# vmskisme/f_renderer

Measured on AMD Instinct MI355X. Metric: Mtri/s (and Mfrag/s), 1M-triangle frame @1920x1080, higher is better.
Workload: dtype f32; 1 GPU; random_1M_tris_1920x1080_depth; scene=1M random clip-space triangles, 1920x1080, depth-only, width=1920, height=1080, triangles=1000000, setup_triangles=1000052, covered_fragments=60715175, varyings=0, tile=32x32, frames_in_flight=2, partition=tile rows in 1 contiguous block(s)

## Files before the change

f_renderer_amd/_native.py:

```python
import ctypes as C
import os
import shutil
import subprocess

_HERE = os.path.dirname(os.path.abspath(__file__))
_ROOT = os.path.dirname(_HERE)
LIB_PATH = os.environ.get("FRR_LIB") or os.path.join(_HERE, "libfrr_hip.so")
_SRC = [os.path.join(_HERE, "csrc", f) for f in ("frr_api.hip", "frr_kernels.h", "frr_raster.h", "frr_device.h", "frr_exact.h", "frr_tile_order.h", "frr_rules.h", "frr_proof.h", "frr_lines.h", "frr_varyings.h", "frr_shade.h", "frr_visible.h", "frr_query.h", "frr_boxes.h", "frr_own.h")]
_HDR = os.path.join(_ROOT, "include", "frr.h")

HIPCC_FLAGS = [
    "--offload-arch=gfx950", "-O3", "-std=c++17", "-fPIC", "-shared",
    "-ffp-contract=off", "-fno-fast-math", "-Wall", "-Wno-unused-function",
    "-fno-slp-vectorize",
    "-DFRR_CSRC_DIR=\"%s\"" % os.path.join(_HERE, "csrc"), "-L/opt/rocm/lib", "-lhiprtc", "-Wl,-rpath,/opt/rocm/lib",
]

FRR_OK, FRR_ERR_INVALID, FRR_ERR_HIP, FRR_ERR_NOMEM, FRR_ERR_UNSUPPORTED, FRR_ERR_CAPACITY = 0, -1, -2, -3, -4, -5
VS_CLIP, VS_CLIP_COLOR, VS_PHONG, VS_GOURAUD = 0, 1, 2, 3
PS_DEPTH, PS_FLAT, PS_COLOR, PS_PHONG, PS_BLINN = 0, 1, 2, 3, 4
CULL_NONE, CULL_NEG, CULL_POS = 0, 1, 2
PER_ITEM, PER_TRIANGLE = 0, 1
VISIBLE_LDS_BINS = 4096
MAX_VARYINGS = 16
# ... 190 lines not shown
```

f_renderer_amd/csrc/frr_api.hip:

```cpp
#include "frr_kernels.h"
#include "frr_tile_order.h"
#include "frr_rules.h"
#include "frr_proof.h"
#include "frr_lines.h"
#include "frr_varyings.h"
#include "frr_shade.h"
#include "frr_visible.h"
#include "frr_query.h"
#include "frr_boxes.h"
#include "frr_own.h"

#include <math.h>
#include <stdio.h>
#include <string.h>
#include <stdlib.h>

#include <hip/hiprtc.h>

#include <map>
#include <mutex>
#include <string>
#include <type_traits>
#include <vector>

// ... 6 lines not shown
FRR_EMBED(frr_src_exact_h, "frr_exact.h");
FRR_EMBED(frr_src_kernels_h, "frr_kernels.h");
FRR_EMBED(frr_src_raster_h, "frr_raster.h");
FRR_EMBED(frr_src_shade_h, "frr_shade.h");
FRR_EMBED(frr_src_visible_h, "frr_visible.h");
FRR_EMBED(frr_src_frr_h, "../../include/frr.h");
#endif
extern "C" const char frr_src_device_h[], frr_src_exact_h[], frr_src_kernels_h[], frr_src_raster_h[], frr_src_shade_h[], frr_src_visible_h[], frr_src_frr_h[];

using namespace frr;
static_assert(PASS_FAN_BITS == FAN_BITS && MAX_PASS_INPUTS << FAN_BITS == 1ull << PASS_ORDER_KEY_BITS, "frr_rules.h: an input's order keys are 32 * input + (0 .. 31), in 32 bits (frr_device.h)");

namespace {

enum KernelId { KID_CLEAR, KID_GEOM, KID_GEOM_SCAN, KID_BIN_COUNT,
                KID_TILE_SCAN, KID_BIN_FILL, KID_RASTER, KID_BIN_SEG, KID_LINES_MARK, KID_LINES_PAINT, KID_VISIBLE, KID_BOXES, KID_COUNT };
const char *const kKernelNames[KID_COUNT] = {"k_clear", "k_geom", "k_geom_scan",
                                             "k_bin_count", "k_tile_scan", "k_bin_fill",
                                             "k_raster", "k_bin_seg", "k_lines_mark", "k_lines_paint", "k_visible", "k_boxes"};

struct Mesh {
    DevBuf<float> own_dev; DevBuf<uint32_t> own_idx;
    const float *dev = nullptr;
    const uint32_t *idx = nullptr;
    uint64_t nverts = 0, ntris = 0;
    bool used = false;
    int vs = 0;
    uint64_t gen = 0;
};
struct Texture {
    DevBuf<uint8_t> dev;
    uint32_t w = 0, h = 0;
};
struct Lines {
// ... 106 lines not shown
    DevBuf<uint4> pbox;
    DevBuf<uint32_t> bcount;
    DevBuf<uint2> clipq;
    DevBuf<float> inst_tab;
    DevBuf<uint32_t> keep_tab;
    DevBuf<uint32_t> vslot[2]; hipStream_t vslot_stream[2] = {nullptr, nullptr};
    uint32_t vslot_seq[2] = {0, 0}, vslot_epoch[2] = {0, 0};
    ReaderFence reader;
};
struct BinSet {
    DevBuf<uint4> bins;
    DevBuf<uint4> bins2;
    DevBuf<uint32_t> bin_matrix;
    DevBuf<uint32_t> tile_cost;
    DevBuf<uint32_t> tile_perm;
    bool cost_known = false; TileOrderKey cost_key = {};
    ReaderFence reader;
};


struct Bound {
    uint8_t *color = nullptr; float *depth = nullptr; uint32_t *tri_id = nullptr;
    int tset = 0;
    int rank = 0, world = 1; bool part_blocked = false;
};
struct Clear {
    bool pending = false;
    bool unowned_debt = false;
    int debt_tiles_y = 0;
    uint32_t rgba = 0; float depth = 0.0f;
// ... 135 lines not shown
    uint32_t lines_chunk = 0;
    DevBuf<uint32_t> vis_bounds[3];
    uint32_t visible_lds_bins = 0;
    DevBuf<uint32_t> box_pyr[3];
    uint32_t box_bounds_chunks = 0;
    ReaderFence wire_reader[2];
    std::map<int, UserModule> user_modules;
    Texture tex[FRR_MAX_TEXTURES];
    frr_uniforms uni;
    DevUniforms duni;
    bool count_frags = true;
    int raster_nw = 0;
    int raster_occ = 0;
    bool raster_sweep = false;
    int tile_order = TILE_ORDER_FIXED;
    uint64_t ordered_passes = 0;
#ifdef FRR_DEBUG_COUNTERS
    DevBuf<unsigned long long> dbg_tiles;
#endif
    Event ev[16];
    bool ev_set[16] = {};
    uint32_t prof_mask = 0;
    std::vector<ProfRec> prof_pending;
    std::vector<Event> ev_pool;
    uint32_t prof_period = 1;
    uint32_t prof_seen[KID_COUNT] = {};
    double prof_ms[KID_COUNT] = {};
    uint32_t prof_n[KID_COUNT] = {};
    std::string err;
};
// ... 636 lines not shown
    a.tiles_x = (int)((ww + TILE - 1) / TILE); a.tiles_y = (int)((wh + TILE - 1) / TILE);
    a.tiles_x_magic = 0u;
    a.own = row_owner(f, a.tiles_y);
    a.recs = S.recs; a.vary = S.vary; a.pbox = S.pbox; a.bcount = S.bcount;
    a.tinfo = S.tinfo; a.fanbase = S.fanbase; a.fan_okey = S.fan_okey; a.block_prefix = S.block_prefix; a.ntris_draw = (uint32_t)f.geom.read.ntris;
    a.tile_counts = c->tile_counts; a.tile_offsets = c->tile_offsets; a.tile_cursor = c->tile_cursor;
    a.gpar = f.gpar(); a.lane = f.lane; a.bpar = 0; a.seq = cmd.seq; a.epoch = c->epoch; a.frame_no = f.frame_no; a.geom_seq = f.geom.seq;
    const uint32_t ntiles = (uint32_t)a.tiles_x * a.tiles_y;
    a.color = f.bound.color; a.depth = f.bound.depth; a.tri_id = f.bound.tri_id; a.cnt = c->cnt;
#ifdef FRR_DEBUG_COUNTERS
    if (!c->dbg_tiles && getenv("FRR_DEBUG_TILES")) (void)c->dbg_tiles.reset((size_t)c->max_tiles * 8);
    if (c->dbg_tiles) (void)hipMemsetAsync(c->dbg_tiles, 0, (size_t)c->max_tiles * 64, tstream_of(c));
    a.dbg_tiles = c->dbg_tiles;
#endif
    a.seg = nullptr; a.nseg = 0;
    a.tile_perm = nullptr; a.tile_cost = nullptr;
    const int owned_rows = a.own.blocked ? a.own.brow1 - a.own.brow0 : (a.tiles_y > f.bound.rank ? (a.tiles_y - f.bound.rank + f.bound.world - 1) / f.bound.world : 0);
    const uint32_t grid = (uint32_t)a.tiles_x * owned_rows;
    if (a.tiles_x >= 2 && a.tiles_x < 65536 && grid < 65536u) a.tiles_x_magic = (uint32_t)(0x100000000ull / (uint64_t)a.tiles_x + 1ull);
    const SpanShape sh = span_shape(c, grid, f.geom.read.ntris, ps_id);
    const bool segmented = grid <= BIN_LDS_MAX_TILES && !c->bin_atomics && !c->raster_sweep;
    const int q = segmented ? (f.bpar() ^ 1) : 0;
    const int bi = !segmented ? 0 : f.geom.on_g ? (f.bset ^ 1) : (frames_alternate(c) ? f.bound.tset : 0);
    BinSet &B = c->bset[bi];
    int rc;
    if (!B.bins) {
        size_t want = std::max<size_t>((size_t)f.geom.read.ntris * 8 + 4 * (size_t)c->max_tiles, (size_t)1 << 22);
        if (c->bin_cap_init) want = c->bin_cap_init;
        want = std::max(want, c->bset[bi ^ 1].bins.cap());
        if ((rc = ensure(c, B.bins, want)) != FRR_OK) return rc;
        if ((rc = ensure(c, B.bins2, want)) != FRR_OK) return rc;
    }
    a.bins2 = B.bins2;
    a.bins = B.bins; a.bin_cap = (uint32_t)std::min<size_t>(B.bins.cap(), 0xFFFFFFFFu);
    hipStream_t gs = gstream_of(c);
    if (segmented) {
        const uint32_t ltiles = std::max<uint32_t>(grid, 1u);
        uint32_t G = (uint32_t)std::min<uint64_t>(std::max<uint64_t>((f.geom.read.ntris + BIN_WG - 1) / BIN_WG, 1), BIN_MAX_G);
        if (c->bin_g > 0) G = (uint32_t)std::min(c->bin_g, BIN_MAX_G);
        G = std::min<uint32_t>(G, sh.nw == 3 ? 256u : (uint32_t)sh.nw * 64u);
        bool fresh_cost;
        if ((rc = ensure(c, B.tile_cost, ltiles, &fresh_cost)) != FRR_OK) return rc;
        if ((rc = ensure(c, B.tile_perm, ltiles)) != FRR_OK) return rc;
        if (fresh_cost) {
            B.cost_known = false;
            HIP_TRY(c, hipMemsetAsync(B.tile_cost, 0, (size_t)ltiles * sizeof(uint32_t), gs));
        }
        const TileOrderKey okey = {grid, a.tiles_x, x0, x1, y0, y1, f.bound.rank, f.bound.world, a.own.blocked, sh.nw};
        const bool ordered = tile_order_built(c->tile_order, c->in_replay, okey, B.cost_known, B.cost_key);
// ... 15 lines not shown
        }
        a.seg = B.bin_matrix; a.nseg = G; a.bpar = q;
        uint64_t SL = std::max<uint64_t>(256, (f.geom.read.ntris * 16 + ntiles - 1) / ntiles);
        SL = std::min<uint64_t>(SL, ((uint64_t)1 << 30) / ltiles);
        if (c->ent_slot_override) SL = c->ent_slot_override;
        a.ent_slot = (uint32_t)SL;
        a.bin_cap = (uint32_t)std::min<size_t>(B.bins.cap(), 0xBFFFFFFFu);
        if ((rc = ensure(c, B.bins2, (size_t)ltiles * SL + a.bin_cap)) != FRR_OK) return rc;
        a.bins2 = B.bins2;
        if ((rc = gstream_wait_readers(c, B.reader)) != FRR_OK) return rc;
        {
            ProfScope p(c, KID_BIN_SEG, gs);
            hipLaunchKernelGGL(k_bin_seg, dim3(G + extra), dim3(BIN_WG), lds, gs, a, ltiles, B.bin_matrix, stage_cap,
                               f.geom.fan_cap, S.block_sums, S.block_prefix, f.geom.nblocks, do_scan | (cmd.query ? 2 : 0), perm_seed);
        }
        if (!cmd.query) { B.cost_known = record; B.cost_key = okey; }
        if (ordered) ++c->ordered_passes;
        f.geom.scan_pending = false;
        f.bpars[f.lane] = q; f.bset = bi;
    } else {
        for (GeomSet &G2 : c->gset) if ((rc = gstream_wait_readers(c, G2.reader)) != FRR_OK) return rc;
        for (BinSet &B2 : c->bset) if ((rc = gstream_wait_readers(c, B2.reader)) != FRR_OK) return rc;
        if ((rc = scan_now(c)) != FRR_OK) return rc;
        const uint32_t bin_grid = (uint32_t)std::min<uint64_t>((f.geom.read.ntris + f.geom.fan_cap + 255) / 256, 2048);
        { ProfScope p(c, KID_BIN_COUNT, gs); hipLaunchKernelGGL(k_bin<false>, dim3(bin_grid), dim3(256), 0, gs, a, f.geom.fan_cap); }
        { ProfScope p(c, KID_TILE_SCAN, gs); if (cmd.query) hipLaunchKernelGGL(k_tile_scan_uncounted, dim3(1), dim3(1024), 0, gs, a, ntiles); else hipLaunchKernelGGL(k_tile_scan, dim3(1), dim3(1024), 0, gs, a, ntiles); }
        { ProfScope p(c, KID_BIN_FILL, gs); hipLaunchKernelGGL(k_bin<true>, dim3(bin_grid), dim3(256), 0, gs, a, f.geom.fan_cap); }
    }
    cmd.par = q; cmd.set = bi; cmd.lane = f.lane;
    HIP_TRY(c, hipGetLastError());
    if (!c->in_replay) {
        const DrawSig sig = draw_sig(f.geom.read, x0, x1, y0, y1, f.bound.rank, f.bound.world, f.bound.part_blocked, f.geom.set, bi, c->join_epoch);
        if (!c->proven.known(sig, f.geom.pred)) {
            HIP_TRY(c, hipEventRecord(c->ev_verify, gs));
            c->verify_pending = true;
            c->verify_pred = f.geom.pred;
            c->verify_sig = sig;
        }
    }
    if ((rc = tstream_wait_gstream(c)) != FRR_OK) return rc;
    if (cmd.query) return launch_query(c, cmd, a, grid, sh, S, B);
    hipStream_t ts;
    if ((rc = target_write(c, !c->in_replay, &ts)) != FRR_OK) return rc;
    const bool shared_entries = ww > (int64_t)x1 && f.bound.world <= 1;
    const int win_safe = a.x0 >= -SPAN_SAFE && a.y0 >= -SPAN_SAFE && a.x1 <= SPAN_SAFE && a.y1 <= SPAN_SAFE;
    if (grid && shared_entries) {
        ProfScope p(c, KID_RASTER, ts);
        const unsigned eg = (unsigned)((((wh - 1) * (int64_t)x1 + ww) + 255) / 256);
        if (um) {
            RasterArgs ra = a; DevUniforms d = cmd.duni;
            void *args[] = {&ra, &d};
            (void)hipModuleLaunchKernel(um->entries, eg, 1, 1, 256, 1, 1, 0, ts, args, nullptr);
        } else {
            switch (ps_id) {
            case FRR_PS_DEPTH: hipLaunchKernelGGL((k_raster_entries<0, FRR_PS_DEPTH>), dim3(eg), dim3(256), 0, ts, a, cmd.duni); break;
            case FRR_PS_FLAT: hipLaunchKernelGGL((k_raster_entries<0, FRR_PS_FLAT>), dim3(eg), dim3(256), 0, ts, a, cmd.duni); break;
            case FRR_PS_COLOR: hipLaunchKernelGGL((k_raster_entries<3, FRR_PS_COLOR>), dim3(eg), dim3(256), 0, ts, a, cmd.duni); break;
            case FRR_PS_PHONG: hipLaunchKernelGGL((k_raster_entries<8, FRR_PS_PHONG>), dim3(eg), dim3(256), 0, ts, a, cmd.duni); break;
            case FRR_PS_BLINN: hipLaunchKernelGGL((k_raster_entries<8, FRR_PS_BLINN>), dim3(eg), dim3(256), 0, ts, a, cmd.duni); break;
            }
// ... 571 lines not shown
    { int rc = finish(c); if (rc != FRR_OK) return rc; }
    c->proven.clear();
    const std::string n(name);
    if (n == "raster_sweep") c->raster_sweep = v != 0;
    else if (n == "raster_nw") { if (v != 0 && v != LIGHT_NW && v != 4 && v != 6 && v != 8 && v != 16) return fail(c, FRR_ERR_INVALID, "raster_nw: 0, 3, 4, 6, 8 or 16"); c->raster_nw = (int)v; }
    else if (n == "raster_occ") { if (v != 0 && v != 4 && v != 6 && v != 8) return fail(c, FRR_ERR_INVALID, "raster_occ: 0, 4, 6 or 8"); c->raster_occ = (int)v; }
    else if (n == "bin_chunks") { if (v < 0) return fail(c, FRR_ERR_INVALID, "bin_chunks >= 0"); c->bin_g = (int)std::min<int64_t>(v, BIN_MAX_G); }
    else if (n == "clear_eager") c->clear_eager = v != 0;
    else if (n == "clip_queue") { if (v < -1 || v > 1) return fail(c, FRR_ERR_INVALID, "clip_queue: -1, 0 or 1"); c->clip_queue = (int)v; }
    else if (n == "tile_slot_records") { if (v < 0 || v > 0x7FFFFFFF) return fail(c, FRR_ERR_INVALID, "tile_slot_records out of range"); c->ent_slot_override = (uint32_t)v; }
    else if (n == "bin_atomics") c->bin_atomics = v != 0;
    else if (n == "bin_capacity") { if (v < 0) return fail(c, FRR_ERR_INVALID, "bin_capacity >= 0"); c->bin_cap_init = (size_t)v; }
    else if (n == "fan_capacity") { if (v < 0) return fail(c, FRR_ERR_INVALID, "fan_capacity >= 0"); c->fan_cap_init = (size_t)v; }
    else if (n == "overlap") { if (v < 0 || v > 2) return fail(c, FRR_ERR_INVALID, "overlap: 0, 1 or 2"); c->overlap = (int)v; }
    else if (n == "bound_targets_in_flight") c->bound_in_flight = v != 0;
    else if (n == "tile_order") { if (v < 0 || v > 2) return fail(c, FRR_ERR_INVALID, "tile_order: 0, 1 or 2"); c->tile_order = (int)v; }
    else if (n == "box_bounds_chunks") { if (v < 0 || v > 1024) return fail(c, FRR_ERR_INVALID, "box_bounds_chunks: 0 .. 1024"); c->box_bounds_chunks = (uint32_t)v; }
    else if (n == "visible_lds_bins") { if (v < 0 || v > (int64_t)VIS_LDS_BINS) return fail(c, FRR_ERR_INVALID, "visible_lds_bins: 0 .. VIS_LDS_BINS"); c->visible_lds_bins = (uint32_t)v; }
    else if (n == "lines_chunk") { if (v < 0 || v > (int64_t)LINES_CHUNK) return fail(c, FRR_ERR_INVALID, "lines_chunk: 0 .. 2^24"); c->lines_chunk = (uint32_t)v; }
    else if (n == "frames_in_flight") { if (v != 1 && v != 2) return fail(c, FRR_ERR_INVALID, "frames_in_flight: 1 or 2"); c->frames_in_flight = (int)v; }
    else return fail(c, FRR_ERR_INVALID, "unknown option");
    return FRR_OK;
}

int frr_set_partition(frr_ctx *c, int rank, int world)
{
    if (!c || world < 1 || rank < 0 || rank >= world) return fail(c, FRR_ERR_INVALID, "bad partition");
    { int rc = settle(c); if (rc != FRR_OK) return rc; }
    c->fs.bound.rank = rank; c->fs.bound.world = world;
    return FRR_OK;
// ... 1363 lines not shown
```

f_renderer_amd/csrc/frr_device.h:

```cpp
#pragma once
#include "../../include/frr.h"
#include "frr_exact.h"

namespace frr {

constexpr int TILE = 32;
constexpr int TILE_PX = TILE * TILE;
constexpr int GEOM_BLOCK = 256;

struct alignas(64) RasterRec {
    uint32_t e[6];
    float s[6];
    float rhw[3];
    uint32_t flags;
};
constexpr int REC_POS_SHIFT = 4, REC_EOFF_SHIFT = 16;
constexpr uint32_t REC_EOFF_MASK = 0x1FFFu;
static_assert(sizeof(RasterRec) == 64, "one cache line per triangle");

#ifdef FRR_DEBUG_COUNTERS
constexpr int DBG_COPIES = 256;
#else
constexpr int DBG_COPIES = 1;
#endif
// ... 125 lines not shown
    int32_t use_clipq;
    uint4 *pbox;
    uint32_t *bcount;
    Counters *cnt;
    const float *inst;
    uint32_t ntris_mesh;
    uint32_t ninst;
    int32_t cull;
    const ListRow *items;
    const uint32_t *item_first;
    const uint32_t *item_ntris;
    const uint32_t *keep;
};

struct RowOwner { int32_t rank, world, blocked, brow0, brow1; };
struct RasterArgs {
    int32_t x0, x1, y0, y1;
    int32_t win_w, win_h;
    int32_t cstride, dstride;
    int32_t tiles_x, tiles_y;
    uint32_t tiles_x_magic;
    RowOwner own;
    const RasterRec *recs;
    const float *vary;
    const uint4 *pbox;
    const uint32_t *bcount;
    const uint32_t *tinfo, *fanbase, *fan_okey, *block_prefix;
    uint32_t ntris_draw;
    uint32_t *tile_counts;
    uint32_t *tile_offsets;
// ... 6 lines not shown
    int32_t lane;
    uint32_t geom_seq;
    int32_t fused_clear;
    uint32_t clear_rgba;
    float clear_depth;
    uint32_t ent_slot;
    uint4 *bins;
    uint4 *bins2;
    uint32_t bin_cap;
    uint32_t *tile_perm;
    uint32_t *tile_cost;
    uint8_t *color;
    float *depth;
    uint32_t *tri_id;
    Counters *cnt;
#ifdef FRR_DEBUG_COUNTERS
    unsigned long long *dbg_tiles;
#endif
};

__device__ __forceinline__ int clampi(int v, int lo, int hi) { return min(max(v, lo), hi); }

FRR_HD bool owns_tile_row(int ty, const RowOwner &o)
{
    return o.world <= 1 || (o.blocked ? (ty >= o.brow0 && ty < o.brow1) : ty % o.world == o.rank);
}

__device__ __forceinline__ int local_tile_row(int ty, const RowOwner &o)
{
    if (o.world <= 1) return ty;
// ... 392 lines not shown
```

f_renderer_amd/csrc/frr_raster.h:

```cpp
#pragma once
#include "frr_device.h"
#ifndef __HIPCC_RTC__
#include <type_traits>
#endif

namespace frr {

__device__ __forceinline__ int xcd_remap(int bid, int nwg)
{
    const int q = nwg / 8, r = nwg % 8, xcd = bid % 8;
    return (xcd < r ? xcd * (q + 1) : r * (q + 1) + (xcd - r) * q) + bid / 8;
}

__device__ __forceinline__ uint32_t order_id(const RasterArgs &a, uint32_t slot)
{
    const uint32_t nt = a.ntris_draw;
    return 1u + (slot < nt ? slot << FAN_BITS : a.fan_okey[slot - nt]);
}
__device__ __forceinline__ uint32_t id_slot(const RasterArgs &a, uint32_t id)
{
    const uint32_t okl = id - 1u, t = okl >> FAN_BITS, f = okl & ((1u << FAN_BITS) - 1u);
    return f ? a.ntris_draw + a.fanbase[t] + (f - 1u) : t;
}
__device__ __forceinline__ uint32_t id_emission(const RasterArgs &a, uint32_t tri_base, uint32_t id)
// ... 383 lines not shown
    const int M = m + __mul24(k, row);
    int q = (int)__builtin_amdgcn_fmed3f((float)M * rD, -2.0f, 40.0f);
    const int r = M - __mul24(q, D);
    q += (r >> 31) + (int)(r >= D);
    lo = max(lo, q & pmask);
    hi = min(hi, max(q + 1, pmask & 64));
}

constexpr int DIRECT_MAX = 256;
#ifndef FRR_DIRECT_STEPS
#define FRR_DIRECT_STEPS 2
#endif
constexpr int DIRECT_STEPS = FRR_DIRECT_STEPS;
constexpr int DIRECT_MIN = 4;
constexpr int HZ_SEG = 0, HZ_BLK = 128, HZ_QUAD = 144, HZ_C4 = 148, HZ_SIZE = 404;
#ifndef FRR_BKT_LOG2
#define FRR_BKT_LOG2 6
#endif
constexpr int BKT_LOG2 = FRR_BKT_LOG2, BKT_N = 1 << BKT_LOG2, BKT_SHIFT = 27 - BKT_LOG2, BKT_PER = BKT_N / 64;
__device__ __forceinline__ uint32_t z_bucket(uint32_t zub_key) { return (uint32_t)(BKT_N - 1) - ((zub_key >> BKT_SHIFT) & (uint32_t)(BKT_N - 1)); }
__device__ __forceinline__ void bucket_scan(uint32_t *s_bkt, int lane, uint32_t base)
{
    uint32_t v[BKT_PER], sum = 0u;
#pragma unroll
    for (int j = 0; j < BKT_PER; ++j) { v[j] = s_bkt[lane * BKT_PER + j]; sum += v[j]; }
    uint32_t run = base + wave_incl_scan_dpp(sum) - sum;
#pragma unroll
    for (int j = 0; j < BKT_PER; ++j) { s_bkt[lane * BKT_PER + j] = run; run += v[j]; }
}
__device__ __forceinline__ uint32_t dpp_xor1(uint32_t v) { return (uint32_t)__builtin_amdgcn_update_dpp(0, (int)v, 0xB1, 0xf, 0xf, false); }
// ... 183 lines not shown
    const uint32_t q = (uint32_t)lane * NW + (uint32_t)w;
    DirectRecs d = {make_uint4(0, 0, 0, 0), q < nent, 0, 0, 64};
    if (d.valid) d.ent = L::exch(lds)[q];
    d.count = __popcll(__ballot(d.valid));
    d.step = max(DIRECT_MIN, (d.count + DIRECT_STEPS - 1) / DIRECT_STEPS);
    __syncthreads();
    return d;
}
__device__ __forceinline__ uint32_t exit_bound(const uint4 &en, int win_safe)
{
    const int mnx = (int)(short)(en.z & 0xFFFFu), mny = (int)(short)(en.z >> 16);
    const int mxx = (int)(short)(en.w & 0xFFFFu), mxy = (int)(short)(en.w >> 16);
    const int amax = max(max(abs(mnx), abs(mxx)), max(abs(mny), abs(mxy)));
    return win_safe && amax <= SPAN_SAFE ? en.y : 0xFFFFFFFFu;
}
template <bool COUNT, int CULL, class L>
__device__ __forceinline__ void span_order_bins2(const RasterArgs &a, const TileCtx &c, unsigned char *lds, uint4 *ents, uint32_t nent, int lane, int w, int win_safe)
{
    constexpr int NW = L::WAVES, B = L::BATCH;
    static_assert(BKT_N >= 64 && DIRECT_MAX * 16 >= 64 * 4, "64 suffix maxima in the bucket counters, 64 step maxima in the exchange buffer");
    const TileSource source = {a, c, a.nseg != 0, L::segpre(lds), L::segsrc(lds)};
    const bool sorted = !COUNT && nent > 2u * B;
    auto bucket_of = [&](const uint4 &e) { return sorted ? z_bucket(e.y) : 0u; };
    uint32_t *gmax = reinterpret_cast<uint32_t *>(L::exch(lds));
    if (!COUNT && threadIdx.x < 64) gmax[threadIdx.x] = 0u;
    auto scatter = [&](const uint4 &en) {
        const uint32_t pos = atomicAdd(&L::bkt(lds)[bucket_of(en)], 1u);
        ents[pos] = en;
        if (!COUNT) atomicMax(&gmax[min((pos - c.beg) / (uint32_t)CULL, 63u)], exit_bound(en, win_safe));
    };
    uint4 ce[4];
#pragma unroll
    for (int k = 0; k < 4; ++k) {
        const uint32_t e = threadIdx.x + (uint32_t)(NW * 64) * k;
        ce[k] = make_uint4(0, 0, 0, 0);
        if (e < nent) { ce[k] = source(e); atomicAdd(&L::bkt(lds)[bucket_of(ce[k])], 1u); }
    }
    for (uint32_t e = threadIdx.x + 4u * NW * 64; e < nent; e += NW * 64) atomicAdd(&L::bkt(lds)[bucket_of(source(e))], 1u);
    __syncthreads();
    if (w == 0) bucket_scan(L::bkt(lds), lane, c.beg);
    __syncthreads();
#pragma unroll
    for (int k = 0; k < 4; ++k) {
        const uint32_t e = threadIdx.x + (uint32_t)(NW * 64) * k;
        if (e < nent) scatter(ce[k]);
    }
    for (uint32_t e = threadIdx.x + 4u * NW * 64; e < nent; e += NW * 64) scatter(source(e));
    __builtin_amdgcn_fence(__ATOMIC_RELEASE, "workgroup");
    __syncthreads();
    __builtin_amdgcn_fence(__ATOMIC_ACQUIRE, "workgroup");
    if (!COUNT) {
        if (w == 0) {
            uint32_t v = gmax[lane];
#pragma unroll
            for (int dd = 1; dd < 64; dd <<= 1) { const uint32_t o = (uint32_t)__shfl_down((int)v, dd, 64); if (lane + dd < 64) v = max(v, o); }
            L::bkt(lds)[lane] = v;
        }
        __syncthreads();
    }
}

struct Culled {
    int bx0, bx1, by0, by1;
    bool alive;
};
template <int PS, bool COUNT, class L>
__device__ __forceinline__ Culled span_cull(const RasterArgs &a, const TileCtx &c, unsigned char *lds, int win_safe, bool valid, const uint4 &en,
                                            int lane, uint32_t &n_cov, uint32_t &n_nan, SpanDbg &dbg)
{
    const int mnx = (int)(short)(en.z & 0xFFFFu), mny = (int)(short)(en.z >> 16);
    const int mxx = (int)(short)(en.w & 0xFFFFu), mxy = (int)(short)(en.w >> 16);
    const int bx0 = max(clampi(mnx, a.x0, a.x1), c.ax0), bx1 = min(clampi(mxx, a.x0, a.x1), c.ax0 + c.tw);
    const int by0 = max(clampi(mny, a.y0, a.y1), c.ay0), by1 = min(clampi(mxy, a.y0, a.y1), c.ay0 + c.th);
    const bool nonempty = valid && bx1 > bx0 && by1 > by0;
// ... 84 lines not shown
    if (len > 0) {
        const uint32_t st = fincl - (uint32_t)len;
        atomicOr(reinterpret_cast<uint32_t *>(&L::hfrag(lds)[w][0]) + (st >> 5), 1u << (st & 31));
        L::q(lds)[w][srank] = (uint32_t)j | ((uint32_t)yl << 5) | (((uint32_t)xl + 2048u - st) << 10);
    }
    wave_lds_fence();
    const unsigned long long hfrag_mine = L::hfrag(lds)[w][lane & 31];
    dbg.fragments(F);
    dbg.T(4);
    return {true, F, hfrag_mine};
}

template <int K, int PS, bool COUNT, int NW, int OCC>
__global__ __launch_bounds__(NW * 64, OCC) void k_raster_span(RasterArgs a, DevUniforms u, int win_safe)
{
    constexpr int B = NW <= 3 ? LIGHT_B : (OCC >= 8 || NW >= 16) ? 16 : SPAN_BATCH;
    constexpr bool TEXTURED = PS == FRR_PS_PHONG || PS == FRR_PS_BLINN || PS >= FRR_SHADER_USER_BASE;
    static_assert(NW >= 3, "the workgroup's threads (three waves: + a second column of wave 0) read all BIN_MAX_G segments; w4[0..3] are all written");
    using L = SpanLds<NW, B>;
    __shared__ __attribute__((aligned(16))) unsigned char lds[L::bytes(TEXTURED)];
    if (TEXTURED) for (int i = threadIdx.x; i < 256; i += NW * 64) L::u8(lds)[i] = (float)i / 255.0f;
    const int lane = threadIdx.x & 63;
    const int w = __builtin_amdgcn_readfirstlane(threadIdx.x >> 6);
    SpanDbg dbg;
    __builtin_amdgcn_s_setprio(3);
    const uint32_t first_bad = seq_first_bad(a.cnt);
    TileCtx c = tile_ctx(a);
    const bool segmented = a.nseg != 0;
    if (!segmented && seq_is_cancelled(first_bad, a.seq, a.epoch, true)) return;
    if (segmented) {
        uint32_t s0 = 0, cn = 0;
        if (threadIdx.x < a.nseg) {
            const uint32_t *r = a.seg + (size_t)threadIdx.x * ((size_t)gridDim.x + 1) + c.ltile;
            s0 = r[0];
            cn = r[1] - s0;
        }
        if (seq_is_cancelled(first_bad, a.seq, a.epoch, true)) return;
        const uint32_t inc = wave_incl_scan_dpp(cn);
        if (lane == 63 && w < 4) L::w4(lds)[w] = inc;
        uint32_t s0x = 0, cnx = 0, incx = 0;
        if (NW == 3 && w == 0) {
            if (192u + (uint32_t)lane < a.nseg) {
                const uint32_t *r = a.seg + (size_t)(192 + lane) * ((size_t)gridDim.x + 1) + c.ltile;
                s0x = r[0];
                cnx = r[1] - s0x;
            }
            incx = wave_incl_scan_dpp(cnx);
            if (lane == 63) L::w4(lds)[3] = incx;
        }
        __syncthreads();
        const uint32_t w0 = L::w4(lds)[0], w1 = L::w4(lds)[1], w2 = L::w4(lds)[2], w3 = L::w4(lds)[3];
        const uint32_t total = __builtin_amdgcn_readfirstlane((w0 + w1) + (w2 + w3));
        if (threadIdx.x == 0 && a.tile_cost) a.tile_cost[c.ltile] = total;
        if (total == 0u) { tile_fill_clear(a, c); return; }
        if (threadIdx.x < BIN_MAX_G) {
            L::segpre(lds)[threadIdx.x] = (w > 0 ? w0 : 0u) + (w > 1 ? w1 : 0u) + (w > 2 ? w2 : 0u) + inc - cn;
            L::segsrc(lds)[threadIdx.x] = s0;
        }
        if (NW == 3 && w == 0) { L::segpre(lds)[192 + lane] = (w0 + w1) + w2 + incx - cnx; L::segsrc(lds)[192 + lane] = s0x; }
        if (threadIdx.x == 0) {
            L::segpre(lds)[BIN_MAX_G] = total;
            const uint32_t ntiles = gridDim.x;
            L::ebase(lds) = total <= a.ent_slot ? (uint32_t)c.ltile * a.ent_slot
                                          : ntiles * a.ent_slot + atomicAdd(&a.cnt->lane[a.lane].btab[a.bpar].ent_cursor, total);
        }
        __syncthreads();
        c.beg = __builtin_amdgcn_readfirstlane(L::ebase(lds));
        c.end = c.beg + total;
    } else if (c.beg >= c.end) {
        tile_fill_clear(a, c);
        return;
    }
    tile_load_keys(a, c, L::key(lds), ~0ull);
    const uint32_t hz0 = a.fused_clear ? zkey_depth(a.clear_depth) : 0u;
    if (threadIdx.x == 0) { L::next(lds) = 0; L::dirty(lds) = a.fused_clear ? 0u : 1u; L::nanflag(lds) = 0u; }
    for (int i = threadIdx.x; i < BKT_N; i += NW * 64) L::bkt(lds)[i] = 0;
    for (int i = threadIdx.x; i < HZ_SIZE; i += NW * 64) L::hz(lds)[i] = i >= HZ_C4 ? hz0 >> 1 : hz0;
    __syncthreads();

    constexpr int CULL = SPAN_CULL < B ? SPAN_CULL : B;
    uint4 *__restrict__ ents = a.bins2;
    const uint32_t nent = c.end - c.beg;
    const bool direct = nent <= (uint32_t)(DIRECT_MAX < NW * 64 ? DIRECT_MAX : NW * 64);
    DirectRecs d = {make_uint4(0, 0, 0, 0), false, 0, 0, 64};
    if (direct) d = span_order_direct<COUNT, L>(a, c, lds, nent, lane, w);
    else span_order_bins2<COUNT, CULL, L>(a, c, lds, ents, nent, lane, w, win_safe);

    __builtin_amdgcn_s_setprio(0);
    const uint32_t le_lo = lane < 32 ? (2u << lane) - 1u : 0xFFFFFFFFu;
    const uint32_t le_hi = lane < 32 ? 0u : (2u << (lane - 32)) - 1u;
    uint32_t n_cov = 0, n_nan = 0;

    if (direct) {
        const int nsteps = max(DIRECT_STEPS, (d.count + B - 1) / B);
        d.step = max(min(DIRECT_MIN, B), (d.count + nsteps - 1) / nsteps);
    }
    if (!COUNT && !direct) dbg.heavy_tile(nent, CULL, w);
    dbg.T(0);
    dbg.main_loop_begins();
    for (;;) {
        uint32_t e0 = 0;
// ... 134 lines not shown
```

f_renderer_amd/renderer.py:

```python
import ctypes as C

import numpy as np

from . import _native as N
from ._native import (CULL_NEG, CULL_NONE, CULL_POS, FrrError, PS_BLINN, PS_COLOR, PS_DEPTH, PS_FLAT, PS_PHONG,
                      VS_CLIP, VS_CLIP_COLOR, VS_GOURAUD, VS_PHONG)

SETUP_DTYPE = np.dtype([("spf", "<f4", (2,)), ("spi", "<i4", (2,)), ("rhw", "<f4"), ("ctx", "<f4", (N.MAX_VARYINGS,))])
assert SETUP_DTYPE.itemsize == C.sizeof(N.SetupVertex)
MATERIAL_DTYPE = np.dtype([("texture_slot", "<i4"), ("ambient_strength", "<f4"), ("specular_strength", "<f4"), ("reserved", "<i4"),
                           ("flat_color", "<f4", (4,)), ("user", "<f4", (N.MATERIAL_USER,))])
assert MATERIAL_DTYPE.itemsize == C.sizeof(N.Material) == 64

_f32p = C.POINTER(C.c_float)


def _fp(a):
    return a.ctypes.data_as(_f32p)



def set_identity():
    m = np.zeros(16, np.float32)
    N.lib().frr_set_identity(_fp(m))
# ... 217 lines not shown


def host_cull_det(clip):
    p = np.ascontiguousarray(clip, np.float32).reshape(12)
    return np.float32(N.lib().frr_host_cull_det(_fp(p)))


def _options_from_env():
    import os
    e, o = os.environ, {}
    if e.get("FRR_RASTER") == "sweep":
        o["raster_sweep"] = 1
    for var, name in (("FRR_RASTER_NW", "raster_nw"), ("FRR_RASTER_OCC", "raster_occ"), ("FRR_BIN_G", "bin_chunks"),
                      ("FRR_ENT_SLOT", "tile_slot_records"), ("FRR_BIN_CAP", "bin_capacity"), ("FRR_FAN_CAP", "fan_capacity"),
                      ("FRR_CLIP_QUEUE", "clip_queue"), ("FRR_OVERLAP", "overlap"), ("FRR_FRAMES_IN_FLIGHT", "frames_in_flight"),
                      ("FRR_BOUND_IN_FLIGHT", "bound_targets_in_flight"), ("FRR_TILE_ORDER", "tile_order")):
        if e.get(var):
            o[name] = int(e[var])
    if e.get("FRR_CLEAR") == "eager":
        o["clear_eager"] = 1
    if e.get("FRR_BIN") == "atomics":
        o["bin_atomics"] = 1
    return o


class Renderer:

    def __init__(self, width, height, device=0, stream=None):
        self._lib = N.lib()
        self.width, self.height = int(width), int(height)
        ctx = C.c_void_p()
# ... 452 lines not shown
```

Measured before the change: 11070 Mtri/s.

## Add tile presort kernel to bucket heavy tiles before rasterization

Adds a k_tile_presort kernel on the geometry stream that does the per-tile prefix of segment counts, depth-bucket sort and per-chunk exit-bound suffix max. It writes the results and a per-tile header into a new tile_hdr buffer. The raster kernel then reads the header and skips its own segment scan and span_order_bins2 for presorted tiles. The aim is to take sorting work out of the LDS- and occupancy-limited raster kernel and let it overlap with other frames' rasterization. The cost is an extra launch and an extra global pass over the entries. It only runs for uncounted, non-query, builtin-shader segmented passes where the triangle density rule holds.

```diff
diff --git a/f_renderer_amd/_native.py b/f_renderer_amd/_native.py
--- a/f_renderer_amd/_native.py
+++ b/f_renderer_amd/_native.py
@@ -6,7 +6,7 @@
 _HERE = os.path.dirname(os.path.abspath(__file__))
 _ROOT = os.path.dirname(_HERE)
 LIB_PATH = os.environ.get("FRR_LIB") or os.path.join(_HERE, "libfrr_hip.so")
-_SRC = [os.path.join(_HERE, "csrc", f) for f in ("frr_api.hip", "frr_kernels.h", "frr_raster.h", "frr_device.h", "frr_exact.h", "frr_tile_order.h", "frr_rules.h", "frr_proof.h", "frr_lines.h", "frr_varyings.h", "frr_shade.h", "frr_visible.h", "frr_query.h", "frr_boxes.h", "frr_own.h")]
+_SRC = [os.path.join(_HERE, "csrc", f) for f in ("frr_api.hip", "frr_kernels.h", "frr_raster.h", "frr_device.h", "frr_exact.h", "frr_tile_order.h", "frr_presort.h", "frr_rules.h", "frr_proof.h", "frr_lines.h", "frr_varyings.h", "frr_shade.h", "frr_visible.h", "frr_query.h", "frr_boxes.h", "frr_own.h")]
 _HDR = os.path.join(_ROOT, "include", "frr.h")
 
 HIPCC_FLAGS = [
diff --git a/f_renderer_amd/csrc/frr_api.hip b/f_renderer_amd/csrc/frr_api.hip
--- a/f_renderer_amd/csrc/frr_api.hip
+++ b/f_renderer_amd/csrc/frr_api.hip
@@ -1,5 +1,6 @@
 #include "frr_kernels.h"
 #include "frr_tile_order.h"
+#include "frr_presort.h"
 #include "frr_rules.h"
 #include "frr_proof.h"
 #include "frr_lines.h"
@@ -44,10 +45,10 @@
 namespace {
 
 enum KernelId { KID_CLEAR, KID_GEOM, KID_GEOM_SCAN, KID_BIN_COUNT,
-                KID_TILE_SCAN, KID_BIN_FILL, KID_RASTER, KID_BIN_SEG, KID_LINES_MARK, KID_LINES_PAINT, KID_VISIBLE, KID_BOXES, KID_COUNT };
+                KID_TILE_SCAN, KID_BIN_FILL, KID_RASTER, KID_BIN_SEG, KID_LINES_MARK, KID_LINES_PAINT, KID_VISIBLE, KID_BOXES, KID_PRESORT, KID_COUNT };
 const char *const kKernelNames[KID_COUNT] = {"k_clear", "k_geom", "k_geom_scan",
                                              "k_bin_count", "k_tile_scan", "k_bin_fill",
-                                             "k_raster", "k_bin_seg", "k_lines_mark", "k_lines_paint", "k_visible", "k_boxes"};
+                                             "k_raster", "k_bin_seg", "k_lines_mark", "k_lines_paint", "k_visible", "k_boxes", "k_presort"};
 
 struct Mesh {
     DevBuf<float> own_dev; DevBuf<uint32_t> own_idx;
@@ -184,6 +185,7 @@
     DevBuf<uint32_t> bin_matrix;
     DevBuf<uint32_t> tile_cost;
     DevBuf<uint32_t> tile_perm;
+    DevBuf<uint32_t> tile_hdr;
     bool cost_known = false; TileOrderKey cost_key = {};
     ReaderFence reader;
 };
@@ -349,6 +351,7 @@
     int raster_occ = 0;
     bool raster_sweep = false;
     int tile_order = TILE_ORDER_FIXED;
+    int tile_presort = TILE_PRESORT_RULE;
     uint64_t ordered_passes = 0;
 #ifdef FRR_DEBUG_COUNTERS
     DevBuf<unsigned long long> dbg_tiles;
@@ -1015,7 +1018,7 @@
     a.dbg_tiles = c->dbg_tiles;
 #endif
     a.seg = nullptr; a.nseg = 0;
-    a.tile_perm = nullptr; a.tile_cost = nullptr;
+    a.tile_perm = nullptr; a.tile_cost = nullptr; a.tile_hdr = nullptr;
     const int owned_rows = a.own.blocked ? a.own.brow1 - a.own.brow0 : (a.tiles_y > f.bound.rank ? (a.tiles_y - f.bound.rank + f.bound.world - 1) / f.bound.world : 0);
     const uint32_t grid = (uint32_t)a.tiles_x * owned_rows;
     if (a.tiles_x >= 2 && a.tiles_x < 65536 && grid < 65536u) a.tiles_x_magic = (uint32_t)(0x100000000ull / (uint64_t)a.tiles_x + 1ull);
@@ -1034,6 +1037,8 @@
     }
     a.bins2 = B.bins2;
     a.bins = B.bins; a.bin_cap = (uint32_t)std::min<size_t>(B.bins.cap(), 0xFFFFFFFFu);
+    const bool shared_entries = ww > (int64_t)x1 && f.bound.world <= 1;
+    const int win_safe = a.x0 >= -SPAN_SAFE && a.y0 >= -SPAN_SAFE && a.x1 <= SPAN_SAFE && a.y1 <= SPAN_SAFE;
     hipStream_t gs = gstream_of(c);
     if (segmented) {
         const uint32_t ltiles = std::max<uint32_t>(grid, 1u);
@@ -1079,6 +1084,13 @@
             hipLaunchKernelGGL(k_bin_seg, dim3(G + extra), dim3(BIN_WG), lds, gs, a, ltiles, B.bin_matrix, stage_cap,
                                f.geom.fan_cap, S.block_sums, S.block_prefix, f.geom.nblocks, do_scan | (cmd.query ? 2 : 0), perm_seed);
         }
+        const PresortPass pp = {true, um == nullptr, cmd.count_frags, cmd.query, grid != 0u && !shared_entries, f.geom.read.ntris, grid, (uint32_t)span_direct_max(sh.nw)};
+        if (tile_presort_runs(c->tile_presort, pp)) {
+            if ((rc = ensure(c, B.tile_hdr, (size_t)ltiles * TILE_HDR_WORDS)) != FRR_OK) return rc;
+            ProfScope p(c, KID_PRESORT, gs);
+            hipLaunchKernelGGL(k_tile_presort, dim3(grid), dim3(256), 0, gs, a, B.tile_hdr.get(), win_safe, (uint32_t)span_cull(sh.nw, sh.occ), pp.direct_max);
+            a.tile_hdr = B.tile_hdr;
+        }
         if (!cmd.query) { B.cost_known = record; B.cost_key = okey; }
         if (ordered) ++c->ordered_passes;
         f.geom.scan_pending = false;
@@ -1107,8 +1119,6 @@
     if (cmd.query) return launch_query(c, cmd, a, grid, sh, S, B);
     hipStream_t ts;
     if ((rc = target_write(c, !c->in_replay, &ts)) != FRR_OK) return rc;
-    const bool shared_entries = ww > (int64_t)x1 && f.bound.world <= 1;
-    const int win_safe = a.x0 >= -SPAN_SAFE && a.y0 >= -SPAN_SAFE && a.x1 <= SPAN_SAFE && a.y1 <= SPAN_SAFE;
     if (grid && shared_entries) {
         ProfScope p(c, KID_RASTER, ts);
         const unsigned eg = (unsigned)((((wh - 1) * (int64_t)x1 + ww) + 255) / 256);
@@ -1710,6 +1720,7 @@
     else if (n == "fan_capacity") { if (v < 0) return fail(c, FRR_ERR_INVALID, "fan_capacity >= 0"); c->fan_cap_init = (size_t)v; }
     else if (n == "overlap") { if (v < 0 || v > 2) return fail(c, FRR_ERR_INVALID, "overlap: 0, 1 or 2"); c->overlap = (int)v; }
     else if (n == "bound_targets_in_flight") c->bound_in_flight = v != 0;
+    else if (n == "tile_presort") { if (v < 0 || v > 2) return fail(c, FRR_ERR_INVALID, "tile_presort: 0, 1 or 2"); c->tile_presort = (int)v; }
     else if (n == "tile_order") { if (v < 0 || v > 2) return fail(c, FRR_ERR_INVALID, "tile_order: 0, 1 or 2"); c->tile_order = (int)v; }
     else if (n == "box_bounds_chunks") { if (v < 0 || v > 1024) return fail(c, FRR_ERR_INVALID, "box_bounds_chunks: 0 .. 1024"); c->box_bounds_chunks = (uint32_t)v; }
     else if (n == "visible_lds_bins") { if (v < 0 || v > (int64_t)VIS_LDS_BINS) return fail(c, FRR_ERR_INVALID, "visible_lds_bins: 0 .. VIS_LDS_BINS"); c->visible_lds_bins = (uint32_t)v; }
diff --git a/f_renderer_amd/csrc/frr_device.h b/f_renderer_amd/csrc/frr_device.h
--- a/f_renderer_amd/csrc/frr_device.h
+++ b/f_renderer_amd/csrc/frr_device.h
@@ -163,6 +163,7 @@
 };
 
 struct RowOwner { int32_t rank, world, blocked, brow0, brow1; };
+constexpr int TILE_HDR_WORDS = 4 + 64;
 struct RasterArgs {
     int32_t x0, x1, y0, y1;
     int32_t win_w, win_h;
@@ -199,6 +200,7 @@
     float *depth;
     uint32_t *tri_id;
     Counters *cnt;
+    const uint32_t *tile_hdr;
 #ifdef FRR_DEBUG_COUNTERS
     unsigned long long *dbg_tiles;
 #endif
diff --git a/f_renderer_amd/csrc/frr_presort.h b/f_renderer_amd/csrc/frr_presort.h
--- /dev/null
+++ b/f_renderer_amd/csrc/frr_presort.h
@@ -0,0 +1,31 @@
+#pragma once
+#include <stdint.h>
+
+namespace frr {
+
+enum TilePresort { TILE_PRESORT_OFF = 0, TILE_PRESORT_ON = 1, TILE_PRESORT_RULE = 2 };
+
+struct PresortPass {
+    bool segmented;
+    bool builtin_shader;
+    bool counted;
+    bool query;
+    bool tile_kernel;
+    uint64_t ntris;
+    uint32_t grid;
+    uint32_t direct_max;
+};
+
+inline bool tile_presort_legal(const PresortPass &p)
+{
+    return p.segmented && p.builtin_shader && !p.counted && !p.query && p.tile_kernel && p.grid != 0u;
+}
+
+inline bool tile_presort_runs(int option, const PresortPass &p)
+{
+    if (option == TILE_PRESORT_OFF || !tile_presort_legal(p)) return false;
+    if (option == TILE_PRESORT_ON) return true;
+    return p.ntris * 2u > (uint64_t)p.direct_max * p.grid;
+}
+
+}
diff --git a/f_renderer_amd/csrc/frr_raster.h b/f_renderer_amd/csrc/frr_raster.h
--- a/f_renderer_amd/csrc/frr_raster.h
+++ b/f_renderer_amd/csrc/frr_raster.h
@@ -421,6 +421,9 @@
 constexpr int DIRECT_STEPS = FRR_DIRECT_STEPS;
 constexpr int DIRECT_MIN = 4;
 constexpr int HZ_SEG = 0, HZ_BLK = 128, HZ_QUAD = 144, HZ_C4 = 148, HZ_SIZE = 404;
+FRR_HD constexpr int span_batch(int nw, int occ) { return nw <= 3 ? LIGHT_B : (occ >= 8 || nw >= 16) ? 16 : SPAN_BATCH; }
+FRR_HD constexpr int span_cull(int nw, int occ) { return SPAN_CULL < span_batch(nw, occ) ? SPAN_CULL : span_batch(nw, occ); }
+FRR_HD constexpr int span_direct_max(int nw) { return DIRECT_MAX < nw * 64 ? DIRECT_MAX : nw * 64; }
 #ifndef FRR_BKT_LOG2
 #define FRR_BKT_LOG2 6
 #endif
@@ -634,6 +637,18 @@
     const int amax = max(max(abs(mnx), abs(mxx)), max(abs(mny), abs(mxy)));
     return win_safe && amax <= SPAN_SAFE ? en.y : 0xFFFFFFFFu;
 }
+__device__ __forceinline__ void scatter_record(uint32_t *s_bkt, uint32_t *gmax, uint4 *ents, const uint4 &en, uint32_t bkt, uint32_t beg, uint32_t cull, int win_safe, bool fold)
+{
+    const uint32_t pos = atomicAdd(&s_bkt[bkt], 1u);
+    ents[pos] = en;
+    if (fold) atomicMax(&gmax[min((pos - beg) / cull, 63u)], exit_bound(en, win_safe));
+}
+__device__ __forceinline__ uint32_t suffix_max64(uint32_t v, int lane)
+{
+#pragma unroll
+    for (int dd = 1; dd < 64; dd <<= 1) { const uint32_t o = (uint32_t)__shfl_down((int)v, dd, 64); if (lane + dd < 64) v = max(v, o); }
+    return v;
+}
 template <bool COUNT, int CULL, class L>
 __device__ __forceinline__ void span_order_bins2(const RasterArgs &a, const TileCtx &c, unsigned char *lds, uint4 *ents, uint32_t nent, int lane, int w, int win_safe)
 {
@@ -644,11 +659,7 @@
     auto bucket_of = [&](const uint4 &e) { return sorted ? z_bucket(e.y) : 0u; };
     uint32_t *gmax = reinterpret_cast<uint32_t *>(L::exch(lds));
     if (!COUNT && threadIdx.x < 64) gmax[threadIdx.x] = 0u;
-    auto scatter = [&](const uint4 &en) {
-        const uint32_t pos = atomicAdd(&L::bkt(lds)[bucket_of(en)], 1u);
-        ents[pos] = en;
-        if (!COUNT) atomicMax(&gmax[min((pos - c.beg) / (uint32_t)CULL, 63u)], exit_bound(en, win_safe));
-    };
+    auto scatter = [&](const uint4 &en) { scatter_record(L::bkt(lds), gmax, ents, en, bucket_of(en), c.beg, (uint32_t)CULL, win_safe, !COUNT); };
     uint4 ce[4];
 #pragma unroll
     for (int k = 0; k < 4; ++k) {
@@ -670,14 +681,59 @@
     __syncthreads();
     __builtin_amdgcn_fence(__ATOMIC_ACQUIRE, "workgroup");
     if (!COUNT) {
-        if (w == 0) {
-            uint32_t v = gmax[lane];
-#pragma unroll
-            for (int dd = 1; dd < 64; dd <<= 1) { const uint32_t o = (uint32_t)__shfl_down((int)v, dd, 64); if (lane + dd < 64) v = max(v, o); }
-            L::bkt(lds)[lane] = v;
-        }
+        if (w == 0) L::bkt(lds)[lane] = suffix_max64(gmax[lane], lane);
         __syncthreads();
     }
+}
+
+__global__ __launch_bounds__(256) void k_tile_presort(RasterArgs a, uint32_t *tile_hdr, int win_safe, uint32_t cull, uint32_t direct_max)
+{
+    static_assert(BIN_MAX_G == 256 && LIGHT_NW * 64 > 2 * LIGHT_B && 4 * 64 > 2 * SPAN_BATCH, "one segment per thread; a heavy tile is always bucketed");
+    __shared__ uint32_t s_segpre[BIN_MAX_G + 4], s_segsrc[BIN_MAX_G], s_bkt[BKT_N], s_gmax[64], s_w4[4], s_ebase;
+    const int lane = threadIdx.x & 63;
+    const int w = __builtin_amdgcn_readfirstlane(threadIdx.x >> 6);
+    const uint32_t first_bad = seq_first_bad(a.cnt);
+    const TileCtx c = tile_ctx(a);
+    uint32_t s0 = 0, cn = 0;
+    if (threadIdx.x < a.nseg) {
+        const uint32_t *r = a.seg + (size_t)threadIdx.x * ((size_t)gridDim.x + 1) + c.ltile;
+        s0 = r[0];
+        cn = r[1] - s0;
+    }
+    if (seq_is_cancelled(first_bad, a.seq, a.epoch, true)) return;
+    const uint32_t inc = wave_incl_scan_dpp(cn);
+    if (lane == 63) s_w4[w] = inc;
+    __syncthreads();
+    const uint32_t w0 = s_w4[0], w1 = s_w4[1], w2 = s_w4[2], w3 = s_w4[3];
+    const uint32_t total = __builtin_amdgcn_readfirstlane((w0 + w1) + (w2 + w3));
+    uint32_t *hdr = tile_hdr + (size_t)c.ltile * TILE_HDR_WORDS;
+    if (total <= direct_max) {
+        if (threadIdx.x == 0) *reinterpret_cast<uint4 *>(hdr) = make_uint4(0u, total, 0u, 0u);
+        return;
+    }
+    s_segpre[threadIdx.x] = (w > 0 ? w0 : 0u) + (w > 1 ? w1 : 0u) + (w > 2 ? w2 : 0u) + inc - cn;
+    s_segsrc[threadIdx.x] = s0;
+    if (threadIdx.x < 64) s_gmax[threadIdx.x] = 0u;
+    for (int i = threadIdx.x; i < BKT_N; i += 256) s_bkt[i] = 0u;
+    if (threadIdx.x == 0) {
+        s_segpre[BIN_MAX_G] = total;
+        s_ebase = total <= a.ent_slot ? (uint32_t)c.ltile * a.ent_slot
+                                      : gridDim.x * a.ent_slot + atomicAdd(&a.cnt->lane[a.lane].btab[a.bpar].ent_cursor, total);
+    }
+    __syncthreads();
+    const uint32_t beg = __builtin_amdgcn_readfirstlane(s_ebase);
+    const TileSource source = {a, c, true, s_segpre, s_segsrc};
+    for (uint32_t e = threadIdx.x; e < total; e += 256u) atomicAdd(&s_bkt[z_bucket(source(e).y)], 1u);
+    __syncthreads();
+    if (w == 0) bucket_scan(s_bkt, lane, beg);
+    __syncthreads();
+    for (uint32_t e = threadIdx.x; e < total; e += 256u) {
+        const uint4 en = source(e);
+        scatter_record(s_bkt, s_gmax, a.bins2, en, z_bucket(en.y), beg, cull, win_safe, true);
+    }
+    __syncthreads();
+    if (w == 0) hdr[4 + lane] = suffix_max64(s_gmax[lane], lane);
+    if (threadIdx.x == 0) *reinterpret_cast<uint4 *>(hdr) = make_uint4(beg, total, 1u, 0u);
 }
 
 struct Culled {
@@ -792,7 +848,7 @@
 template <int K, int PS, bool COUNT, int NW, int OCC>
 __global__ __launch_bounds__(NW * 64, OCC) void k_raster_span(RasterArgs a, DevUniforms u, int win_safe)
 {
-    constexpr int B = NW <= 3 ? LIGHT_B : (OCC >= 8 || NW >= 16) ? 16 : SPAN_BATCH;
+    constexpr int B = span_batch(NW, OCC);
     constexpr bool TEXTURED = PS == FRR_PS_PHONG || PS == FRR_PS_BLINN || PS >= FRR_SHADER_USER_BASE;
     static_assert(NW >= 3, "the workgroup's threads (three waves: + a second column of wave 0) read all BIN_MAX_G segments; w4[0..3] are all written");
     using L = SpanLds<NW, B>;
@@ -813,38 +869,56 @@
             s0 = r[0];
             cn = r[1] - s0;
         }
+        uint4 hd = make_uint4(0u, 0u, 0u, 0u);
+        uint32_t hsuf = 0u;
+        if constexpr (!COUNT) {
+            if (a.tile_hdr) {
+                const uint32_t *h = a.tile_hdr + (size_t)c.ltile * TILE_HDR_WORDS;
+                hd = *reinterpret_cast<const uint4 *>(h);
+                if (threadIdx.x < 64) hsuf = h[4 + threadIdx.x];
+            }
+        }
         if (seq_is_cancelled(first_bad, a.seq, a.epoch, true)) return;
-        const uint32_t inc = wave_incl_scan_dpp(cn);
-        if (lane == 63 && w < 4) L::w4(lds)[w] = inc;
-        uint32_t s0x = 0, cnx = 0, incx = 0;
-        if (NW == 3 && w == 0) {
-            if (192u + (uint32_t)lane < a.nseg) {
-                const uint32_t *r = a.seg + (size_t)(192 + lane) * ((size_t)gridDim.x + 1) + c.ltile;
-                s0x = r[0];
-                cnx = r[1] - s0x;
+        bool presorted = false;
+        if constexpr (!COUNT) presorted = __builtin_amdgcn_readfirstlane(hd.z) != 0u;
+        if (presorted) {
+            c.beg = __builtin_amdgcn_readfirstlane(hd.x);
+            c.end = c.beg + __builtin_amdgcn_readfirstlane(hd.y);
+            if (threadIdx.x < 64) L::bkt(lds)[threadIdx.x] = hsuf;
+            if (threadIdx.x == 0 && a.tile_cost) a.tile_cost[c.ltile] = c.end - c.beg;
+        } else {
+            const uint32_t inc = wave_incl_scan_dpp(cn);
+            if (lane == 63 && w < 4) L::w4(lds)[w] = inc;
+            uint32_t s0x = 0, cnx = 0, incx = 0;
+            if (NW == 3 && w == 0) {
+                if (192u + (uint32_t)lane < a.nseg) {
+                    const uint32_t *r = a.seg + (size_t)(192 + lane) * ((size_t)gridDim.x + 1) + c.ltile;
+                    s0x = r[0];
+                    cnx = r[1] - s0x;
+                }
+                incx = wave_incl_scan_dpp(cnx);
+                if (lane == 63) L::w4(lds)[3] = incx;
             }
-            incx = wave_incl_scan_dpp(cnx);
-            if (lane == 63) L::w4(lds)[3] = incx;
-        }
-        __syncthreads();
-        const uint32_t w0 = L::w4(lds)[0], w1 = L::w4(lds)[1], w2 = L::w4(lds)[2], w3 = L::w4(lds)[3];
-        const uint32_t total = __builtin_amdgcn_readfirstlane((w0 + w1) + (w2 + w3));
-        if (threadIdx.x == 0 && a.tile_cost) a.tile_cost[c.ltile] = total;
-        if (total == 0u) { tile_fill_clear(a, c); return; }
-        if (threadIdx.x < BIN_MAX_G) {
-            L::segpre(lds)[threadIdx.x] = (w > 0 ? w0 : 0u) + (w > 1 ? w1 : 0u) + (w > 2 ? w2 : 0u) + inc - cn;
-            L::segsrc(lds)[threadIdx.x] = s0;
-        }
-        if (NW == 3 && w == 0) { L::segpre(lds)[192 + lane] = (w0 + w1) + w2 + incx - cnx; L::segsrc(lds)[192 + lane] = s0x; }
-        if (threadIdx.x == 0) {
-            L::segpre(lds)[BIN_MAX_G] = total;
-            const uint32_t ntiles = gridDim.x;
-            L::ebase(lds) = total <= a.ent_slot ? (uint32_t)c.ltile * a.ent_slot
-                                          : ntiles * a.ent_slot + atomicAdd(&a.cnt->lane[a.lane].btab[a.bpar].ent_cursor, total);
-        }
-        __syncthreads();
-        c.beg = __builtin_amdgcn_readfirstlane(L::ebase(lds));
-        c.end = c.beg + total;
+            __syncthreads();
+            const uint32_t w0 = L::w4(lds)[0], w1 = L::w4(lds)[1], w2 = L::w4(lds)[2], w3 = L::w4(lds)[3];
+            const uint32_t total = __builtin_amdgcn_readfirstlane((w0 + w1) + (w2 + w3));
+            if (threadIdx.x == 0 && a.tile_cost) a.tile_cost[c.ltile] = total;
+            if (total == 0u) { tile_fill_clear(a, c); return; }
+            if (threadIdx.x < BIN_MAX_G) {
+                L::segpre(lds)[threadIdx.x] = (w > 0 ? w0 : 0u) + (w > 1 ? w1 : 0u) + (w > 2 ? w2 : 0u) + inc - cn;
+                L::segsrc(lds)[threadIdx.x] = s0;
+            }
+            if (NW == 3 && w == 0) { L::segpre(lds)[192 + lane] = (w0 + w1) + w2 + incx - cnx; L::segsrc(lds)[192 + lane] = s0x; }
+            if (threadIdx.x == 0) {
+                L::segpre(lds)[BIN_MAX_G] = total;
+                const uint32_t ntiles = gridDim.x;
+                L::ebase(lds) = total <= a.ent_slot ? (uint32_t)c.ltile * a.ent_slot
+                                              : ntiles * a.ent_slot + atomicAdd(&a.cnt->lane[a.lane].btab[a.bpar].ent_cursor, total);
+            }
+            __syncthreads();
+            c.beg = __builtin_amdgcn_readfirstlane(L::ebase(lds));
+            c.end = c.beg + total;
+        }
     } else if (c.beg >= c.end) {
         tile_fill_clear(a, c);
         return;
@@ -852,17 +926,22 @@
     tile_load_keys(a, c, L::key(lds), ~0ull);
     const uint32_t hz0 = a.fused_clear ? zkey_depth(a.clear_depth) : 0u;
     if (threadIdx.x == 0) { L::next(lds) = 0; L::dirty(lds) = a.fused_clear ? 0u : 1u; L::nanflag(lds) = 0u; }
-    for (int i = threadIdx.x; i < BKT_N; i += NW * 64) L::bkt(lds)[i] = 0;
+    if constexpr (COUNT) {
+        for (int i = threadIdx.x; i < BKT_N; i += NW * 64) L::bkt(lds)[i] = 0;
+    } else {
+        const bool direct0 = c.end - c.beg <= (uint32_t)span_direct_max(NW);
+        if (direct0 || !a.tile_hdr) for (int i = threadIdx.x; i < BKT_N; i += NW * 64) L::bkt(lds)[i] = 0;
+    }
     for (int i = threadIdx.x; i < HZ_SIZE; i += NW * 64) L::hz(lds)[i] = i >= HZ_C4 ? hz0 >> 1 : hz0;
     __syncthreads();
 
-    constexpr int CULL = SPAN_CULL < B ? SPAN_CULL : B;
+    constexpr int CULL = span_cull(NW, OCC);
     uint4 *__restrict__ ents = a.bins2;
     const uint32_t nent = c.end - c.beg;
-    const bool direct = nent <= (uint32_t)(DIRECT_MAX < NW * 64 ? DIRECT_MAX : NW * 64);
+    const bool direct = nent <= (uint32_t)span_direct_max(NW);
     DirectRecs d = {make_uint4(0, 0, 0, 0), false, 0, 0, 64};
     if (direct) d = span_order_direct<COUNT, L>(a, c, lds, nent, lane, w);
-    else span_order_bins2<COUNT, CULL, L>(a, c, lds, ents, nent, lane, w, win_safe);
+    else if (COUNT || !a.tile_hdr) span_order_bins2<COUNT, CULL, L>(a, c, lds, ents, nent, lane, w, win_safe);
 
     __builtin_amdgcn_s_setprio(0);
     const uint32_t le_lo = lane < 32 ? (2u << lane) - 1u : 0xFFFFFFFFu;
diff --git a/f_renderer_amd/renderer.py b/f_renderer_amd/renderer.py
--- a/f_renderer_amd/renderer.py
+++ b/f_renderer_amd/renderer.py
@@ -255,7 +255,8 @@
     for var, name in (("FRR_RASTER_NW", "raster_nw"), ("FRR_RASTER_OCC", "raster_occ"), ("FRR_BIN_G", "bin_chunks"),
                       ("FRR_ENT_SLOT", "tile_slot_records"), ("FRR_BIN_CAP", "bin_capacity"), ("FRR_FAN_CAP", "fan_capacity"),
                       ("FRR_CLIP_QUEUE", "clip_queue"), ("FRR_OVERLAP", "overlap"), ("FRR_FRAMES_IN_FLIGHT", "frames_in_flight"),
-                      ("FRR_BOUND_IN_FLIGHT", "bound_targets_in_flight"), ("FRR_TILE_ORDER", "tile_order")):
+                      ("FRR_BOUND_IN_FLIGHT", "bound_targets_in_flight"), ("FRR_TILE_ORDER", "tile_order"),
+                      ("FRR_TILE_PRESORT", "tile_presort")):
         if e.get(var):
             o[name] = int(e[var])
     if e.get("FRR_CLEAR") == "eager":
```

Result: slower. 10800 Mtri/s (-2.5%).
